# agent-charon/MinGraph-UNet

Measured on AMD Instinct MI355X. Metric: segmented Mpix/sec, full MinGraph-UNet forward (U-Net + patch-graph GAT), 512x512 batch, higher is better.
Workload: dtype f32

## Files before the change

### mingraph-unet_amd/csrc/common.h

```cpp
#pragma once
#include <hip/hip_runtime.h>
#include <stdint.h>

#include "device.h"

namespace mgu {

inline int grid_for(int64_t work, int threads, int cap) {
  int64_t b = (work + threads - 1) / threads;
  if (b < 1) b = 1;
  if (b > cap) b = cap;
  return (int)b;
}
inline bool aligned16(const void* p) { return ((uintptr_t)p & 15) == 0; }

struct Tuning {
  bool first_mfma = true;
  bool use_wino = true;
  int wino_prec = 1;
  bool convt_frag = true;
  bool wino_cp = true;
  int wino_ppb_cap = 32;
  bool wgrad_halo = true;
  bool wino_wgrad = true;
  bool convt_dgrad_x3 = true;
  bool wgrad_x3 = true;
  bool wgrad_thin = true;
  bool wino_dgrad = true;
  bool gat_fused = true;
  bool head_fused = true;
  bool wino_asm = true;
};
const Tuning& default_tuning();
hipError_t ensure_dyn_lds(const void* func, size_t bytes, bool (&done)[64]);

struct IgemmDesc {
  const Tuning* tn;
  const float* in;
  const float* w;
  const float* wu;
  const float* scale;
  const float* shift;
  float* out;
  int M;
  int H, W;
  int Cp;
  int ldin;
  int KS;
  int K;
  int Kp;
  int N;
  int ldout;
  int coff;
  int relu;
  int out_mode;
  int ct_cout;
  int Hout, Wout;
  float* pool;
  int ldpool;
  double* stat_slots;
  int split_n;
  float* out2;
  int ld2;
};

struct WinoHead {
  const float* w;
  const float* b;
  float* logits;
  float* psum;
  int ncls;
  int psum_bytes;
};
inline size_t wino_head_psum_bytes(int B, int H, int W) { return (size_t)B * (H / 16) * (W / 16) * 8 * 32 * sizeof(float); }

inline const Tuning& tun(const IgemmDesc& d) { return d.tn ? *d.tn : default_tuning(); }
enum class ConvKernel {
  None,
  WinoAsmWide, WinoAsmCp1r2, WinoAsmCp1r4,
  WinoAsmCp1r2Head,
  WinoCp2, WinoCp1, WinoCp2Stats, WinoCp1Stats,
  WinoCp1Head,
  WinoF32Wide, WinoF32Narrow,
  WinoX3Wide, WinoX3Narrow,
  HaloF32, HaloBf16Np8, HaloBf16Np4,
  TilesF32, TilesBf16,
  ConvtX3, ConvtBf16f, ConvtX3Dgrad,
};
ConvKernel pick_conv(const IgemmDesc& d, int dtype, const WinoHead* head = nullptr);
hipError_t launch_conv(const IgemmDesc& d, ConvKernel k, int dtype, hipStream_t s, const WinoHead* head = nullptr);
inline bool conv_fuses_head(ConvKernel k) { return k == ConvKernel::WinoAsmCp1r2Head || k == ConvKernel::WinoCp1Head; }
inline hipError_t launch_igemm_f32(const IgemmDesc& d, hipStream_t s) { return launch_conv(d, pick_conv(d, 0), 0, s); }
inline hipError_t launch_igemm_bf16(const IgemmDesc& d, hipStream_t s) { return launch_conv(d, pick_conv(d, 1), 1, s); }
const char* conv_kernel_name(ConvKernel k, const IgemmDesc& d);
const char* conv_dgrad_name(ConvKernel k, const IgemmDesc& d);
struct ConvCost {
  double mfma;
  int pipe;
};
ConvCost conv_cost(ConvKernel k, const IgemmDesc& d);
inline bool conv_is_wino(ConvKernel k) { return k >= ConvKernel::WinoAsmWide && k <= ConvKernel::WinoX3Narrow; }
inline bool conv_fuses_pool(ConvKernel k) {
  return conv_is_wino(k) || (k >= ConvKernel::HaloF32 && k <= ConvKernel::HaloBf16Np4);
}
inline bool conv_reads_panel(ConvKernel k) {
  return !conv_is_wino(k) && k != ConvKernel::ConvtX3 && k != ConvKernel::ConvtBf16f && k != ConvKernel::ConvtX3Dgrad;
}
bool wino_layer(const Tuning& t, int KS, int Cp);
bool wino_dgrad_layer(const Tuning& t, int KS, int Cop);
bool convt_x3_layer(const Tuning& t, int Cin, int Cout);
bool convt_x3_dgrad_layer(const Tuning& t, int Cin, int Cout);
bool convt_bf16f_layer(const Tuning& t, int Cin, int Cout);
bool wino_head_layer(const Tuning& t, int dtype, int Cin, int ncls, int patch, int B, int H, int W);
inline bool wino_wide(const IgemmDesc& d) { return d.N > 32; }
// ... 157 lines not shown
```

### mingraph-unet_amd/csrc/ctx.h

```cpp
#pragma once
#include <stdarg.h>
#include <stdio.h>
#include <stdlib.h>
#include <string.h>

#include <map>
#include <string>
#include <vector>

#include "../../include/mgunet.h"
#include "common.h"

struct Layer {
  std::string prefix;
  std::string conv;
  std::string bn;
  int Cin = 0, Cp = 0, Cout = 0, KS = 3;
  bool convt = false;
  int K = 0, Kp = 0, N = 0, Np = 0;
  float *wp = nullptr, *scale = nullptr, *shift = nullptr;
  bool first = false;
  bool ctb = false;
  bool ctx3 = false;
  bool wino = false;
// ... 11 lines not shown
  float *mean = nullptr, *invstd = nullptr, *tscale = nullptr, *tshift = nullptr;
  const float* t_in = nullptr;
  int t_ldin = 0;
  float* t_z = nullptr;
  float* t_y = nullptr;
  int t_ldy = 0;
  int t_B = 0, t_H = 0, t_W = 0;
  int level = 0;
};

struct Block {
  int up = -1;
  int conv1 = 0, conv2 = 0;
  int level = 0;
};

struct mgu_ctx {
  int device = 0;
  mgu::Tuning tn;
  std::string err;
  bool configured = false, loaded = false;
  std::vector<mgu::PackBatch> pack_host;
  mgu::PackBatch* pack_dev = nullptr;
  int pack_dev_cap = 0;
  bool want_train = false;
  bool fold_dirty = false;
  int* err_word = nullptr;
  void* redws = nullptr;
  size_t redws_bytes = 0;
  int last_stat_rows = 0;
  void* pm_out = nullptr;
  int pm_patch = 0;
  void* pmws = nullptr;
  size_t pmws_bytes = 0;
  void* wuws = nullptr;
  size_t wuws_bytes = 0;
  unsigned long long* gmaxbuf = nullptr;
  int gmax_cap = 0;
  unsigned gmax_gen = 0;
  struct mgu_gat_weights* gat_tmp = nullptr;
  void* lossws = nullptr;
  size_t lossws_bytes = 0;
  void* imgws = nullptr;
  size_t imgws_bytes = 0;
  void* ncws = nullptr;
  size_t ncws_bytes = 0;
  void* objws = nullptr;
  size_t objws_bytes = 0;
  int in_ch = 0, ncls = 0, feat = 0, depth = 0, dtype = 0, Cp0 = 0;
  std::vector<Layer> layers;
  std::vector<Block> enc, dec;
  Block bott;
  int head = 0;
  int64_t nparams = 0;
  float* arena = nullptr;
  size_t arena_floats = 0;
  void* ws = nullptr;
  size_t ws_bytes = 0;
  void* gbws = nullptr;
  size_t gbws_bytes = 0;
  void* gws = nullptr;
  size_t gws_bytes = 0;
  void* tws = nullptr;
  size_t tws_bytes = 0;
  bool have_train_fwd = false;
  int tB = 0, tH = 0, tW = 0;
  std::vector<float*> t_cat, t_feat, t_pooled;
  float* t_logits = nullptr;
  void* comm = nullptr;
  int comm_world = 1, comm_rank = 0;
  hipStream_t comm_stream = nullptr;
  hipEvent_t comm_ev[16] = {};
  int comm_ev_next = 0;
  bool prof = false;
  std::vector<hipEvent_t> ev;
  struct ProfRec {
    const char* name;
    double alg, mfma;
    int pipe;
  };
  std::vector<ProfRec> prec;
  int ev_used = 0;
  hipEvent_t ev_total[2] = {nullptr, nullptr};
};

namespace mgud {

inline int rup(int v, int m) { return (v + m - 1) / m * m; }
extern std::string g_create_err;

inline int fail(mgu_ctx* c, int code, const char* fmt, ...) {
  char buf[512];
  va_list ap;
  va_start(ap, fmt);
  vsnprintf(buf, sizeof buf, fmt, ap);
  va_end(ap);
  if (c) c->err = buf; else g_create_err = buf;
  return code;
}

#define HIPCHK(c, call)                                                                                       \
  do {                                                                                                        \
    hipError_t e_ = (call);                                                                                   \
    if (e_ != hipSuccess) return mgud::fail(c, MGU_ERR_HIP, "%s failed: %s", #call, hipGetErrorString(e_));   \
  } while (0)

inline int ensure(mgu_ctx* c, void** p, size_t* have, size_t need) {
  if (*have >= need) return MGU_OK;
  if (*p) {
    HIPCHK(c, hipDeviceSynchronize());
    HIPCHK(c, hipFree(*p));
    *p = nullptr;
    *have = 0;
  }
  hipError_t e = hipMalloc(p, need);
  if (e != hipSuccess) return fail(c, MGU_ERR_NOMEM, "hipMalloc(%zu) failed: %s", need, hipGetErrorString(e));
  *have = need;
  return MGU_OK;
}

inline int err_word_dev(mgu_ctx* c, int** dev) {
  if (!c->err_word) {
    HIPCHK(c, hipHostMalloc((void**)&c->err_word, sizeof(int), hipHostMallocMapped));
    *c->err_word = 0;
  }
  HIPCHK(c, hipHostGetDevicePointer((void**)dev, c->err_word, 0));
  return MGU_OK;
}
inline const char* err_word_message(int w) {
  return (w & 2) ? "the GAT backward found no edge whose score equals the forward's graph-wide maximum (mgu_gat_layer_backward): its "
                   "max term was not applied"
                 : "a label outside [0, num_classes) (and != ignore_index -100) reached a loss kernel of this context (mgu_cross_entropy / "
                   "mgu_dice_loss; F.one_hot / CrossEntropyLoss raise on it)";
}

struct Carve {
  size_t off = 0;
  size_t take(size_t bytes) {
    const size_t o = off;
    off += (bytes + 255) / 256 * 256;
    return o;
  }
};

struct ProfScope {
  mgu_ctx* c;
  hipStream_t s;
  int idx = -1;
  ProfScope(mgu_ctx* c_, hipStream_t s_, const char* name = "conv/GEMM", double alg = 0, double mfma = 0, int pipe = -1) : c(c_), s(s_) {
    if (!c || !c->prof) return;
    if ((size_t)c->ev_used >= c->prec.size()) c->prec.resize(c->ev_used + 1);
    c->prec[c->ev_used] = {name, alg, mfma, pipe};
    if ((size_t)(2 * c->ev_used + 2) > c->ev.size()) {
      hipEvent_t a, b;
      if (hipEventCreate(&a) != hipSuccess || hipEventCreate(&b) != hipSuccess) return;
      c->ev.push_back(a);
      c->ev.push_back(b);
    }
    idx = c->ev_used++;
    (void)hipEventRecord(c->ev[2 * idx], s);
  }
  ~ProfScope() {
    if (idx >= 0) (void)hipEventRecord(c->ev[2 * idx + 1], s);
  }
};

// ... 112 lines not shown
```

### mingraph-unet_amd/csrc/mgunet_api.hip

```cpp
#include "ctx.h"

#include <algorithm>

using namespace mgu;
using namespace mgud;

namespace mgud {
std::string g_create_err;
}

namespace {

struct WsPlan {
  size_t xin, tmp, bott, total;
  std::vector<size_t> pooled;
};

WsPlan plan_ws(const mgu_ctx* c, int B, int H, int W) {
  std::vector<int> hs, wsz;
  level_dims(H, W, c->depth, hs, wsz);
  auto out = [&](const Block& b, int l) { return (size_t)B * hs[l] * wsz[l] * c->layers[b.conv2].Cout; };
  WsPlan p;
  Carve k;
  const size_t es = c->dtype == MGU_DTYPE_BF16 ? 2 : 4;
  p.xin = k.take((size_t)B * H * W * c->Cp0 * es);
  size_t tmax = out(c->bott, c->bott.level);
  for (const Block& b : c->enc) tmax = std::max(tmax, out(b, b.level));
  p.tmp = k.take(tmax * es);
  for (const Block& b : c->enc) p.pooled.push_back(k.take(out(b, b.level + 1) * es));
  p.bott = k.take(out(c->bott, c->bott.level) * es);
  p.total = k.off;
  return p;
}

template <class F>
void weight_forms(const mgu_ctx* c, Layer& L, F form) {
  const int dtype = c->dtype;
  L.wino = dtype == MGU_DTYPE_F32 && !L.convt && wino_layer(c->tn, L.KS, L.Cp);
  L.ctx3 = dtype == MGU_DTYPE_F32 && L.convt && convt_x3_layer(c->tn, L.Cin, L.Cout);
  L.ctb = dtype == MGU_DTYPE_BF16 && L.convt && convt_bf16f_layer(c->tn, L.Cin, L.Cout);
  L.first = !L.convt && L.KS == 3 && first_conv_applicable(dtype, L.Cin, L.Cp, L.Cout, 8, 0);
  form(L.wp, (size_t)L.Np * L.Kp);
  form(L.scale, (size_t)L.Np);
  form(L.shift, (size_t)L.Np);
  if (L.wino) form(L.wu, wino_u_floats(L.Cout, L.Cp));
  if (L.wino && rup(L.Cout, 4) % 16 == 0) form(L.wug, wino_u_floats(L.Cin, rup(L.Cout, 4)));
  if (L.ctx3) form(L.wu, convt_x3_floats(L.Cin, L.Cout));
  if (L.ctb) form(L.wu, convt_bf16f_floats(L.Cin, L.Cout));
  if (L.ctx3) form(L.wxg, convt_x3_dgrad_floats(L.Cin, L.Cout));
  if (dtype == MGU_DTYPE_F32 && !L.convt && L.bn.empty())
    form(L.wxg, (size_t)rup(L.Cin, 128) * rup(L.KS * L.KS * rup(L.Cout, 4), 32));
  if (L.first) form(L.wf, 9 * 4 * (size_t)L.Cout);
  if (L.first) form(L.wfm, first_mfma_floats());
  if (!L.bn.empty()) {
    form(L.mean, (size_t)L.Np);
    form(L.invstd, (size_t)L.Np);
    form(L.tscale, (size_t)L.Np);
    form(L.tshift, (size_t)L.Np);
  }
}

}

extern "C" {

const char* mgu_version(void) { return "mgunet 0.2 (gfx950: fp32 Winograd / bf16 MFMA forward, fp32 training step, GAT, RCCL gradient exchange)"; }

int mgu_create(int device_id, mgu_ctx** out) {
  if (!out) return fail(nullptr, MGU_ERR_INVALID, "out == NULL");
  int n = 0;
  hipError_t e = hipGetDeviceCount(&n);
  if (e != hipSuccess || n <= 0)
    return fail(nullptr, MGU_ERR_HIP, "no HIP device available (%s): libmgunet has no CPU fallback",
                e != hipSuccess ? hipGetErrorString(e) : "device count 0");
  if (device_id < 0 || device_id >= n) return fail(nullptr, MGU_ERR_INVALID, "device %d out of range [0,%d)", device_id, n);
  e = hipSetDevice(device_id);
  if (e != hipSuccess) return fail(nullptr, MGU_ERR_HIP, "hipSetDevice: %s", hipGetErrorString(e));
  mgu_ctx* c = new mgu_ctx();
  c->device = device_id;
  auto flag = [](const char* name) { const char* v = getenv(name); return v && v[0] == '1'; };
  auto num = [](const char* name, int dflt) { const char* v = getenv(name); return v && v[0] ? atoi(v) : dflt; };
  Tuning& t = c->tn;
  t.first_mfma = !flag("MGU_NO_FIRST_MFMA");
  t.use_wino = !flag("MGU_NO_WINOGRAD");
  t.wino_prec = num("MGU_WINO_PREC", t.wino_prec) ? 1 : 0;
  t.wino_cp = !flag("MGU_NO_WINO_CP");
  t.convt_frag = !flag("MGU_NO_CONVT_FRAG");
  t.wino_ppb_cap = std::max(1, num("MGU_WINO_PPB_CAP", 32));
  t.wgrad_halo = !flag("MGU_NO_WGRAD_HALO");
  t.wino_wgrad = !flag("MGU_NO_WINO_WGRAD");
  t.wgrad_x3 = !flag("MGU_NO_WGRAD_X3");
  t.convt_dgrad_x3 = !flag("MGU_NO_CONVT_DGRAD_X3");
  t.wgrad_thin = !flag("MGU_NO_THIN_WGRAD");
  t.wino_dgrad = !flag("MGU_NO_WINO_DGRAD");
  t.gat_fused = !flag("MGU_NO_GAT_FUSED");
  t.wino_asm = num("MGU_WINO_ASM", 1) > 0;
  t.head_fused = num("MGU_HEAD_FUSED", 1) > 0;
  *out = c;
  return MGU_OK;
}

void mgu_destroy(mgu_ctx* c) {
  if (!c) return;
  (void)hipSetDevice(c->device);
  (void)hipDeviceSynchronize();
  (void)mgu_comm_destroy(c);
  if (c->arena) (void)hipFree(c->arena);
  if (c->ws) (void)hipFree(c->ws);
  if (c->gws) (void)hipFree(c->gws);
  if (c->pmws) (void)hipFree(c->pmws);
  if (c->gbws) (void)hipFree(c->gbws);
  if (c->pack_dev) (void)hipFree(c->pack_dev);
  if (c->tws) (void)hipFree(c->tws);
  if (c->redws) (void)hipFree(c->redws);
  if (c->wuws) (void)hipFree(c->wuws);
  if (c->ncws) (void)hipFree(c->ncws);
  if (c->objws) (void)hipFree(c->objws);
  if (c->lossws) (void)hipFree(c->lossws);
  if (c->imgws) (void)hipFree(c->imgws);
  gat_destroy(c);
  if (c->err_word) (void)hipHostFree(c->err_word);
  for (auto e : c->ev) (void)hipEventDestroy(e);
  for (auto e : c->ev_total)
    if (e) (void)hipEventDestroy(e);
  delete c;
}

const char* mgu_last_error(mgu_ctx* c) { return c ? c->err.c_str() : g_create_err.c_str(); }

int mgu_unet_configure(mgu_ctx* c, int in_ch, int ncls, int feat, int depth, int dtype) {
  if (!c) return MGU_ERR_INVALID;
  if (in_ch < 1 || ncls < 1 || feat < 4 || (feat & 3) || depth < 1 || depth > 8)
    return fail(c, MGU_ERR_INVALID, "unsupported UNet(%d,%d,%d,%d): init_features must be a positive multiple of 4, depth 1..8",
                in_ch, ncls, feat, depth);
  if (dtype != MGU_DTYPE_F32 && dtype != MGU_DTYPE_BF16) return fail(c, MGU_ERR_INVALID, "unknown dtype %d", dtype);
  if (dtype == MGU_DTYPE_BF16 && ((feat & 7) || ncls > 4))
    return fail(c, MGU_ERR_INVALID, "bf16 storage needs init_features %% 8 == 0 (16-byte lanes of 8 bf16) and <= 4 classes");
  HIPCHK(c, hipSetDevice(c->device));
  c->in_ch = in_ch, c->ncls = ncls, c->feat = feat, c->depth = depth, c->dtype = dtype;
  c->Cp0 = rup(in_ch, dtype == MGU_DTYPE_BF16 ? 8 : 4);
  c->layers.clear();
  c->enc.clear();
  c->dec.clear();
  auto add = [&](const std::string& prefix, const char* conv, const char* bn, int cin, int cp, int cout, int KS, bool convt, int level) {
    Layer L;
    L.prefix = prefix, L.conv = conv, L.bn = bn;
    L.Cin = cin, L.Cp = cp, L.Cout = cout, L.KS = KS, L.convt = convt, L.level = level;
    c->layers.push_back(L);
    return (int)c->layers.size() - 1;
  };
  auto add_block = [&](const std::string& prefix, int cin, int cp, int cout, int level, int up) {
    Block b;
    b.up = up, b.level = level;
    b.conv1 = add(prefix, "conv1", "bn1", cin, cp, cout, 3, false, level);
    b.conv2 = add(prefix, "conv2", "bn2", cout, cout, cout, 3, false, level);
    return b;
  };
  int cin = in_ch, cp = c->Cp0, f = feat;
  for (int i = 0; i < depth; ++i) {
    c->enc.push_back(add_block("encoder.encoder_blocks." + std::to_string(i) + ".", cin, cp, f, i, -1));
    cin = cp = f;
    f *= 2;
  }
  c->bott = add_block("encoder.bottleneck.", cin, cp, f, depth, -1);
  int prev = f;
  for (int b = 0; b < depth; ++b) {
    const int i = depth - 1 - b, ci = feat << i;
    const std::string prefix = "decoder.decoder_blocks." + std::to_string(b) + ".";
    const int up = add(prefix, "upsample", "", prev, prev, prev / 2, 1, true, i + 1);
    c->dec.push_back(add_block(prefix + "conv_block.", ci + prev / 2, ci + prev / 2, ci, i, up));
    prev = ci;
  }
  c->head = add("decoder.", "final_conv", "", prev, prev, ncls, 1, false, 0);
  for (auto& L : c->layers) {
    L.K = L.KS * L.KS * L.Cp;
    L.Kp = rup(L.K, dtype == MGU_DTYPE_BF16 ? 64 : 32);
    L.N = L.convt ? 4 * L.Cout : L.Cout;
    L.Np = rup(L.N, 128);
  }
  {
    int64_t off = 0;
    auto conv = [&](Layer& L) {
      L.off_w = off, off += (int64_t)L.Cout * L.Cin * L.KS * L.KS * (L.convt ? 4 : 1);
      L.off_b = off, off += L.Cout;
    };
    auto bn = [&](Layer& L) {
      L.off_gamma = off, off += L.Cout;
      L.off_beta = off, off += L.Cout;
    };
    auto block = [&](const Block& b) {
      if (b.up >= 0) conv(c->layers[b.up]);
      conv(c->layers[b.conv1]), conv(c->layers[b.conv2]);
      bn(c->layers[b.conv1]), bn(c->layers[b.conv2]);
    };
    for (const Block& b : c->enc) block(b);
    block(c->bott);
    for (const Block& b : c->dec) block(b);
    conv(c->layers[c->head]);
    c->nparams = off;
  }
  size_t total = 0;
  for (auto& L : c->layers) weight_forms(c, L, [&](float*&, size_t n) { total += n; });
  if (c->arena) HIPCHK(c, hipFree(c->arena));
  c->arena = nullptr;
  HIPCHK(c, hipMalloc((void**)&c->arena, total * sizeof(float)));
  HIPCHK(c, hipMemset(c->arena, 0, total * sizeof(float)));
  c->arena_floats = total;
// ... 119 lines not shown
        items.push_back(pack_wino(w, L.wug, L.Cin, L.Cout, rup(L.Cout, 4), 1, c->tn.wino_prec));
        L.wug_valid = true;
      }
      const bool head_kernel = L.bn.empty() && c->ncls <= 4;
      if (!L.wu && !L.first && !head_kernel) {
        items.push_back(pack_conv_panel(w, L.wp, c->dtype, L.Cout, L.Cin, L.Cp, L.KS, L.Kp));
        L.wp_dirty = false;
      }
      if (L.wf) items.push_back(pack_first_w(w, L.wf, L.Cout, L.Cin));
      if (L.wfm && L.Cout == 32 && L.Cin <= 3) items.push_back(pack_first_mfma(w, L.wfm, L.Cout, L.Cin));
      if (!L.bn.empty()) c->fold_dirty = true;
      else items.push_back(pack_bias_tile(b, L.shift, L.Cout, 1));
      if (L.bn.empty() && L.wxg && c->want_train) {
        const int Cop = rup(L.Cout, 4);
        items.push_back(pack_dgrad_panel(w, L.wxg, L.Cout, L.Cin, Cop, L.KS, rup(L.KS * L.KS * Cop, 32)));
        L.wxg_valid = true;
      }
    }
  }
  std::vector<PackBatch> batches;
  for (size_t i0 = 0; i0 < items.size(); i0 += PACK_MAX) {
    PackBatch b;
    memset(&b, 0, sizeof b);
    b.n = (int)std::min<size_t>(PACK_MAX, items.size() - i0);
    for (int i = 0; i < b.n; ++i) b.it[i] = items[i0 + i];
    if (!pack_batch_prepare(b)) return fail(c, MGU_ERR_STATE, "internal: a weight form is not packable");
    batches.push_back(b);
  }
  const bool same = batches.size() == c->pack_host.size() &&
                    (batches.empty() || memcmp(batches.data(), c->pack_host.data(), batches.size() * sizeof(PackBatch)) == 0);
  if (!same) {
    if ((int)batches.size() > c->pack_dev_cap) {
      if (c->pack_dev) HIPCHK(c, hipFree(c->pack_dev));
      c->pack_dev = nullptr;
      HIPCHK(c, hipMalloc((void**)&c->pack_dev, batches.size() * sizeof(PackBatch)));
      c->pack_dev_cap = (int)batches.size();
    }
    HIPCHK(c, hipStreamSynchronize(s));
    HIPCHK(c, hipMemcpy(c->pack_dev, batches.data(), batches.size() * sizeof(PackBatch), hipMemcpyHostToDevice));
    c->pack_host = batches;
  }
  for (size_t k = 0; k < batches.size(); ++k) HIPCHK(c, launch_pack_batch(c->pack_dev + k, batches[k].total_blocks, s));
  return MGU_OK;
}

int mgud::run_layer(mgu_ctx* c, const Layer& L, const void* in_v, int ldin, int B, int H, int W, void* out_v, int ldout,
                    int coff, int relu, const float* scale, const float* shift, int Hout, int Wout, hipStream_t s,
                    void* pool, int ldpool, bool* pool_fused, double* stat_slots, bool* stat_fused, const WinoHead* head,
                    bool* head_fused) {
  IgemmDesc d = layer_desc(c, L, in_v, ldin, B, H, W, out_v, ldout, coff);
  if (head_fused) *head_fused = false;
  d.scale = scale, d.shift = shift, d.relu = relu, d.Hout = Hout, d.Wout = Wout;
  if (pool_fused) *pool_fused = false;
  if (stat_fused) *stat_fused = false;
  if (L.wfm && c->tn.first_mfma && ldin == L.Cp && first_mfma_applicable(c->dtype, L.Cin, L.Cp, L.Cout, ldout, coff, H, W)) {
    const double alg = 2.0 * d.M * 9.0 * L.Cin * L.Cout;
    ProfScope ps(c, s, "conv3x3_first_mfma_kernel", alg, 2.0 * d.M * 32.0 * 32.0 * (c->dtype == MGU_DTYPE_F32 ? 6.0 : 3.0), 1);
    HIPCHK(c, launch_first_mfma(c->dtype, in_v, L.wfm, scale, shift, out_v, B, H, W, ldout, coff, relu, s));
    return MGU_OK;
  }
  if (L.wf && ldin == L.Cp && first_conv_applicable(c->dtype, L.Cin, L.Cp, L.Cout, ldout, coff) &&
      (int64_t)B * H * W * std::max(ldout, 8) < (1ll << 31)) {
    ProfScope ps(c, s, "conv3x3_first_kernel", 2.0 * d.M * 9.0 * L.Cin * L.Cout, 0, -1);
    HIPCHK(c, launch_first_conv(c->dtype, in_v, L.wf, scale, shift, out_v, B, H, W, L.Cin, L.Cout, ldout, coff, relu, s));
    return MGU_OK;
  }
  ConvKernel k = pick_conv(d, c->dtype, head);
  if (stat_slots && conv_is_wino(k) && wino_grid_blocks(d) <= STAT_ROWS) {
    d.stat_slots = stat_slots;
    c->last_stat_rows = wino_grid_blocks(d);
    if (stat_fused) *stat_fused = true;
  }
  if (pool && conv_fuses_pool(k)) {
    d.pool = (float*)pool, d.ldpool = ldpool;
    if (pool_fused) *pool_fused = true;
  }
  if (d.stat_slots || d.pool) k = pick_conv(d, c->dtype, head);
  if (!conv_fuses_head(k)) head = nullptr;
  else if (head_fused) *head_fused = true;
  if (L.wp_dirty && conv_reads_panel(k)) {
    HIPCHK(c, launch_pack_one(L.convt ? pack_convt_panel(L.w_src, L.wp, c->dtype, L.Cin, L.Cout, L.Kp)
                                      : pack_conv_panel(L.w_src, L.wp, c->dtype, L.Cout, L.Cin, L.Cp, L.KS, L.Kp), s));
    L.wp_dirty = false;
  }
  double alg = L.convt ? 2.0 * d.M * (double)L.Cin * L.Cout * 4.0 : 2.0 * d.M * (double)L.KS * L.KS * L.Cin * L.Cout;
  if (head) alg += 2.0 * d.M * (double)L.Cout * head->ncls;
  const ConvCost cost = conv_cost(k, d);
  ProfScope ps(c, s, conv_kernel_name(k, d), alg, cost.mfma, cost.pipe);
  HIPCHK(c, launch_conv(d, k, c->dtype, s, head));
  return MGU_OK;
}

static int run_conv(mgu_ctx* c, const Layer& L, const void* in, int ldin, int B, int H, int W, void* out, int ldout,
                    int coff, int relu, int Hout, int Wout, hipStream_t s, void* pool = nullptr, int ldpool = 0,
                    bool* pool_fused = nullptr, const WinoHead* head = nullptr, bool* head_fused = nullptr) {
  return run_layer(c, L, in, ldin, B, H, W, out, ldout, coff, relu, L.bn.empty() ? nullptr : L.scale, L.shift, Hout, Wout, s,
                   pool, ldpool, pool_fused, nullptr, nullptr, head, head_fused);
}

extern "C" {

int mgu_unet_forward(mgu_ctx* c, const void* x_dev, int B, int H, int W, int64_t xs_n, int64_t xs_c, int64_t xs_h,
                     int64_t xs_w, void* logits_dev, void* const* cat_dev, void* const* feat_dev, int training,
                     void* hip_stream) {
  if (!c) return MGU_ERR_INVALID;
  if (!c->configured || !c->loaded) return fail(c, MGU_ERR_STATE, "configure + load_weights must precede forward");
  if (!x_dev || !logits_dev || !cat_dev || !feat_dev) return fail(c, MGU_ERR_INVALID, "NULL buffer");
  const int depth = c->depth;
  if (B < 1 || H < (1 << depth) || W < (1 << depth))
    return fail(c, MGU_ERR_INVALID, "input %dx%dx%d too small for depth %d", B, H, W, depth);
  if ((int64_t)B * H * W >= (1ll << 31)) return fail(c, MGU_ERR_INVALID, "B*H*W must be < 2^31");
  for (int i = 0; i < depth; ++i)
    if (!cat_dev[i] || !feat_dev[i]) return fail(c, MGU_ERR_INVALID, "NULL cat/feat buffer %d", i);
  HIPCHK(c, hipSetDevice(c->device));
  hipStream_t s = (hipStream_t)hip_stream;
  if (training && c->dtype != MGU_DTYPE_F32)
    return fail(c, MGU_ERR_STATE, "training runs in fp32 only (bf16 storage is an inference mode)");
  if (training) {
    int rc = unet_forward_train(c, (const float*)x_dev, xs_n, xs_c, xs_h, xs_w, B, H, W, (float*)logits_dev, cat_dev, feat_dev, s);
    if (rc == MGU_OK && c->pm_out) {
      ProfScope ps(c, s, "patch_mean_kernel", 0, 0, -1);
      HIPCHK(c, launch_patch_mean(feat_dev[0], 0, (float*)c->pm_out, B, H, W, c->feat, c->pm_patch, s));
      c->pm_out = nullptr;
    }
    return rc;
  }
  const WsPlan plan = plan_ws(c, B, H, W);
  int rc = ensure(c, &c->ws, &c->ws_bytes, plan.total);
  if (rc) return rc;
  const Layer& F = c->layers[c->head];
  WinoHead head_args{};
  bool head_done = false;
  const bool head_wanted = c->pm_out && F.w_src && F.b_src && wino_head_layer(c->tn, c->dtype, F.Cin, c->ncls, c->pm_patch, B, H, W);
  if (head_wanted) {
    if ((rc = ensure(c, &c->pmws, &c->pmws_bytes, wino_head_psum_bytes(B, H, W)))) return rc;
    head_args = WinoHead{F.w_src, F.b_src, (float*)logits_dev, (float*)c->pmws, c->ncls, (int)wino_head_psum_bytes(B, H, W)};
  }
  if (c->fold_dirty) {
    for (auto& L : c->layers)
      if (!L.bn.empty()) HIPCHK(c, launch_bn_fold(L.b_src, L.gamma, L.beta, L.run_mean, L.run_var, 1e-5f, L.scale, L.shift, L.Cout, s));
    c->fold_dirty = false;
  }
  char* ws = (char*)c->ws;
  const size_t es = c->dtype == MGU_DTYPE_BF16 ? 2 : 4;
  void* xin = ws + plan.xin;
  void* tmp = ws + plan.tmp;
  void* bott = ws + plan.bott;
  std::vector<int> hs, wsz;
  level_dims(H, W, depth, hs, wsz);

  if (c->prof) {
    for (auto& e : c->ev_total)
      if (!e) HIPCHK(c, hipEventCreate(&e));
    HIPCHK(c, hipEventRecord(c->ev_total[0], s));
  }

  for (const Block& b : c->enc) {
    const int i = b.level;
    if (2 * hs[i + 1] != hs[i] || 2 * wsz[i + 1] != wsz[i])
      HIPCHK(c, hipMemsetAsync(cat_dev[i], 0, (size_t)B * hs[i] * wsz[i] * 2 * c->layers[b.conv2].Cout * es, s));
  }

  const Layer& L0 = c->layers[c->enc[0].conv1];
  const bool first_direct = L0.wfm && c->tn.first_mfma && first_mfma_applicable(c->dtype, L0.Cin, L0.Cp, L0.Cout, c->feat, 0, H, W) &&
                            (int64_t)B * H * W < (1ll << 31);
  if (!first_direct) HIPCHK(c, launch_pack_input((const float*)x_dev, xin, c->dtype, B, c->in_ch, c->Cp0, H, W, xs_n, xs_c, xs_h, xs_w, s));

  const void* cur = xin;
  int cur_ld = c->Cp0;
  for (const Block& b : c->enc) {
    const int i = b.level, C = c->layers[b.conv1].Cout;
    if (&b == &c->enc.front() && first_direct) {
      if (c->fold_dirty) return fail(c, MGU_ERR_STATE, "internal: eval scale/shift not folded");
      const double alg = 2.0 * B * H * W * 9.0 * L0.Cin * L0.Cout;
      ProfScope ps(c, s, "conv3x3_first_mfma_kernel", alg, 2.0 * B * H * W * 32.0 * 32.0 * (c->dtype == MGU_DTYPE_F32 ? 6.0 : 3.0), 1);
      HIPCHK(c, launch_first_mfma_direct(c->dtype, (const float*)x_dev, xs_n, xs_c, xs_h, xs_w, c->in_ch, L0.wfm, L0.bn.empty() ? nullptr : L0.scale,
                                         L0.shift, tmp, B, H, W, C, 0, 1, s));
    } else if ((rc = run_conv(c, c->layers[b.conv1], cur, cur_ld, B, hs[i], wsz[i], tmp, C, 0, 1, 0, 0, s))) return rc;
    void* pooled = ws + plan.pooled[i];
    bool fused = false;
    if ((rc = run_conv(c, c->layers[b.conv2], tmp, C, B, hs[i], wsz[i], cat_dev[i], 2 * C, 0, 1, 0, 0, s, pooled, C, &fused))) return rc;
    if (!fused) HIPCHK(c, launch_maxpool2(cat_dev[i], 2 * C, pooled, c->dtype, B, hs[i], wsz[i], C, s));
    cur = pooled;
    cur_ld = C;
  }
  {
    const Block& b = c->bott;
    const int i = b.level, C = c->layers[b.conv1].Cout;
    if ((rc = run_conv(c, c->layers[b.conv1], cur, cur_ld, B, hs[i], wsz[i], tmp, C, 0, 1, 0, 0, s))) return rc;
    if ((rc = run_conv(c, c->layers[b.conv2], tmp, C, B, hs[i], wsz[i], bott, C, 0, 1, 0, 0, s))) return rc;
    cur = bott;
    cur_ld = C;
  }
  for (const Block& b : c->dec) {
    const int i = b.level, C = c->layers[b.conv1].Cout;
    const bool last = head_wanted && i == 0;
    if ((rc = run_conv(c, c->layers[b.up], cur, cur_ld, B, hs[i + 1], wsz[i + 1], cat_dev[i], 2 * C, C, 0, hs[i], wsz[i], s)))
      return rc;
    if ((rc = run_conv(c, c->layers[b.conv1], cat_dev[i], 2 * C, B, hs[i], wsz[i], tmp, C, 0, 1, 0, 0, s))) return rc;
    if ((rc = run_conv(c, c->layers[b.conv2], tmp, C, B, hs[i], wsz[i], feat_dev[i], C, 0, 1, 0, 0, s, nullptr, 0, nullptr,
                       last ? &head_args : nullptr, last ? &head_done : nullptr)))
      return rc;
    cur = feat_dev[i];
    cur_ld = C;
  }
  {
    const int pm_dtype = c->dtype;
    if (head_done) {
      ProfScope ps(c, s, "patch_sum_combine_kernel", 0, 0, -1);
      HIPCHK(c, launch_patch_sum_combine((const float*)c->pmws, (float*)c->pm_out, B * (H / 16) * (W / 16), s));
      c->pm_out = nullptr;
    } else if (c->pm_out && F.w_src && F.b_src && patch_mean_head_fusable(pm_dtype, F.Cin, c->ncls) && F.Cin <= 256) {
      ProfScope ps(c, s, "patch_mean_kernel (1x1 head + patch means)", 2.0 * B * H * W * F.Cin * c->ncls, 0, -1);
      HIPCHK(c, launch_patch_mean(cur, pm_dtype, (float*)c->pm_out, B, H, W, F.Cin, c->pm_patch, s, F.w_src, F.b_src,
                                  (float*)logits_dev, c->ncls));
      c->pm_out = nullptr;
    } else if (c->ncls <= 4 && F.w_src && F.b_src) {
      ProfScope ps(c, s, "conv1x1_head_kernel", 2.0 * B * H * W * F.Cin * c->ncls, 0, -1);
      HIPCHK(c, launch_conv1x1_head(cur, c->dtype, cur_ld, F.Cin, F.w_src, F.b_src, (float*)logits_dev, c->ncls, c->ncls,
                                    (int64_t)B * H * W, s));
    } else if ((rc = run_conv(c, F, cur, cur_ld, B, H, W, logits_dev, c->ncls, 0, 0, 0, 0, s))) {
      return rc;
    }
  }
  if (c->pm_out) {
    ProfScope ps(c, s, "patch_mean_kernel", 0, 0, -1);
    HIPCHK(c, launch_patch_mean(cur, c->dtype, (float*)c->pm_out, B, H, W, F.Cin, c->pm_patch, s));
    c->pm_out = nullptr;
  }
  if (c->prof) HIPCHK(c, hipEventRecord(c->ev_total[1], s));
  return MGU_OK;
}

int mgu_unet_request_patch_mean(mgu_ctx* c, int patch, void* out_dev) {
  if (!c) return MGU_ERR_INVALID;
  if (!c->configured) return fail(c, MGU_ERR_STATE, "not configured");
  if (!out_dev) {
    c->pm_out = nullptr;
    return MGU_OK;
  }
  if (patch < 1) return fail(c, MGU_ERR_INVALID, "bad patch_mean request");
  const int C = c->layers[c->head].Cin, vec = c->dtype == MGU_DTYPE_BF16 ? 8 : 4;
  if ((C % vec) || C > 256) return fail(c, MGU_ERR_INVALID, "patch means need init_features %% %d == 0 and <= 256 (got %d)", vec, C);
  c->pm_patch = patch;
  c->pm_out = out_dev;
  return MGU_OK;
}

struct mgu_conv_weights {
  Layer L;
};

static Layer block_layer(int Cin, int Cout, int ksize, bool convt) {
  Layer L;
  L.Cin = L.Cp = Cin, L.Cout = Cout, L.KS = ksize, L.convt = convt;
  L.K = ksize * ksize * Cin, L.Kp = rup(L.K, 32), L.N = convt ? 4 * Cout : Cout, L.Np = rup(L.N, 128);
  return L;
}

static int conv2d_launch(mgu_ctx* c, const Layer& L, const void* in_dev, int B, int H, int W, const void* bias_dev, const void* scale_dev,
                         const void* shift_dev, int relu, void* out_dev, int ld_out, int c_off, hipStream_t s) {
  IgemmDesc d = layer_desc(c, L, in_dev, L.Cin, B, H, W, out_dev, ld_out, c_off);
  d.relu = relu;
  if (scale_dev && shift_dev) {
    d.scale = (const float*)scale_dev;
    d.shift = (const float*)shift_dev;
  } else if (bias_dev) {
    HIPCHK(c, launch_pack_one(pack_bias_tile((const float*)bias_dev, L.shift, L.Cout, 1), s));
    d.shift = L.shift;
  }
  const ConvKernel k = pick_conv(d, 0);
  ProfScope ps(c, s, conv_kernel_name(k, d));
  HIPCHK(c, launch_conv(d, k, 0, s));
  return MGU_OK;
}

int mgu_conv2d_prepare(mgu_ctx* c, const void* w_dev, int Cout, int Cin, int ksize, mgu_conv_weights** out, void* hip_stream) {
  if (!c) return MGU_ERR_INVALID;
  if (!w_dev || !out || Cout < 1 || (ksize != 1 && ksize != 3)) return fail(c, MGU_ERR_INVALID, "bad conv2d_prepare args (ksize must be 1 or 3)");
  if (Cin < 4 || (Cin & 3)) return fail(c, MGU_ERR_INVALID, "conv2d needs Cin %% 4 == 0 (got %d)", Cin);
  HIPCHK(c, hipSetDevice(c->device));
  hipStream_t s = (hipStream_t)hip_stream;
  mgu_conv_weights* p = new mgu_conv_weights();
  Layer& L = p->L;
  L = block_layer(Cin, Cout, ksize, false);
  const bool wino = wino_layer(c->tn, ksize, Cin);
  const size_t panel = (size_t)L.Np * L.Kp, total = panel + L.Np + (wino ? wino_u_floats(Cout, Cin) : 0);
  hipError_t e = hipMalloc((void**)&L.wp, total * sizeof(float));
// ... 195 lines not shown
```

Measured before the change: 804.6.

## Split U-Net forward batch into two image groups on concurrent streams

Splits the batch into two halves and runs the encoder/decoder walk for each half on its own stream (the main stream plus a new non-blocking stream), with per-group tmp slices and offset activation pointers, joined by events. The aim is to overlap kernels from the two groups so small, low-occupancy layers at deep levels fill the GPU better and launch gaps are hidden. In exchange each kernel gets half the work, which can lower per-kernel efficiency on the large layers. It also adds event synchronisation, including an extra wait when weight panels are repacked during the first group.

Measured after the change: 821.0, median of 6. +2.0%, better.

```diff
diff --git a/mingraph-unet_amd/csrc/common.h b/mingraph-unet_amd/csrc/common.h
--- a/mingraph-unet_amd/csrc/common.h
+++ b/mingraph-unet_amd/csrc/common.h
@@ -30,6 +30,7 @@
   bool gat_fused = true;
   bool head_fused = true;
   bool wino_asm = true;
+  int fwd_groups = 2;
 };
 const Tuning& default_tuning();
 hipError_t ensure_dyn_lds(const void* func, size_t bytes, bool (&done)[64]);
diff --git a/mingraph-unet_amd/csrc/ctx.h b/mingraph-unet_amd/csrc/ctx.h
--- a/mingraph-unet_amd/csrc/ctx.h
+++ b/mingraph-unet_amd/csrc/ctx.h
@@ -117,6 +117,9 @@
   std::vector<ProfRec> prec;
   int ev_used = 0;
   hipEvent_t ev_total[2] = {nullptr, nullptr};
+  hipStream_t fwd_stream = nullptr;
+  hipEvent_t fwd_ev[2] = {nullptr, nullptr};
+  int panel_packs = 0;
 };
 
 namespace mgud {
diff --git a/mingraph-unet_amd/csrc/mgunet_api.hip b/mingraph-unet_amd/csrc/mgunet_api.hip
--- a/mingraph-unet_amd/csrc/mgunet_api.hip
+++ b/mingraph-unet_amd/csrc/mgunet_api.hip
@@ -12,9 +12,12 @@
 namespace {
 
 struct WsPlan {
-  size_t xin, tmp, bott, total;
+  size_t xin, tmp, tmp_slice, bott, total;
   std::vector<size_t> pooled;
 };
+
+int fwd_groups(const mgu_ctx* c, int B) { return c->tn.fwd_groups >= 2 && B >= 2 ? 2 : 1; }
+int group_images(const mgu_ctx* c, int B) { return (B + fwd_groups(c, B) - 1) / fwd_groups(c, B); }
 
 WsPlan plan_ws(const mgu_ctx* c, int B, int H, int W) {
   std::vector<int> hs, wsz;
@@ -26,7 +29,9 @@
   p.xin = k.take((size_t)B * H * W * c->Cp0 * es);
   size_t tmax = out(c->bott, c->bott.level);
   for (const Block& b : c->enc) tmax = std::max(tmax, out(b, b.level));
-  p.tmp = k.take(tmax * es);
+  const int G = fwd_groups(c, B);
+  p.tmp_slice = (tmax / B * group_images(c, B) * es + 255) / 256 * 256;
+  p.tmp = k.take(G == 1 ? tmax * es : G * p.tmp_slice);
   for (const Block& b : c->enc) p.pooled.push_back(k.take(out(b, b.level + 1) * es));
   p.bott = k.take(out(c->bott, c->bott.level) * es);
   p.total = k.off;
@@ -96,6 +101,7 @@
   t.gat_fused = !flag("MGU_NO_GAT_FUSED");
   t.wino_asm = num("MGU_WINO_ASM", 1) > 0;
   t.head_fused = num("MGU_HEAD_FUSED", 1) > 0;
+  t.fwd_groups = num("MGU_FWD_GROUPS", t.fwd_groups) >= 2 ? 2 : 1;
   *out = c;
   return MGU_OK;
 }
@@ -123,6 +129,9 @@
   for (auto e : c->ev) (void)hipEventDestroy(e);
   for (auto e : c->ev_total)
     if (e) (void)hipEventDestroy(e);
+  for (auto e : c->fwd_ev)
+    if (e) (void)hipEventDestroy(e);
+  if (c->fwd_stream) (void)hipStreamDestroy(c->fwd_stream);
   delete c;
 }
 
@@ -408,6 +417,7 @@
     HIPCHK(c, launch_pack_one(L.convt ? pack_convt_panel(L.w_src, L.wp, c->dtype, L.Cin, L.Cout, L.Kp)
                                       : pack_conv_panel(L.w_src, L.wp, c->dtype, L.Cout, L.Cin, L.Cp, L.KS, L.Kp), s));
     L.wp_dirty = false;
+    ++c->panel_packs;
   }
   double alg = L.convt ? 2.0 * d.M * (double)L.Cin * L.Cout * 4.0 : 2.0 * d.M * (double)L.KS * L.KS * L.Cin * L.Cout;
   if (head) alg += 2.0 * d.M * (double)L.Cout * head->ncls;
@@ -470,7 +480,6 @@
   char* ws = (char*)c->ws;
   const size_t es = c->dtype == MGU_DTYPE_BF16 ? 2 : 4;
   void* xin = ws + plan.xin;
-  void* tmp = ws + plan.tmp;
   void* bott = ws + plan.bott;
   std::vector<int> hs, wsz;
   level_dims(H, W, depth, hs, wsz);
@@ -492,44 +501,79 @@
                             (int64_t)B * H * W < (1ll << 31);
   if (!first_direct) HIPCHK(c, launch_pack_input((const float*)x_dev, xin, c->dtype, B, c->in_ch, c->Cp0, H, W, xs_n, xs_c, xs_h, xs_w, s));
 
-  const void* cur = xin;
-  int cur_ld = c->Cp0;
-  for (const Block& b : c->enc) {
-    const int i = b.level, C = c->layers[b.conv1].Cout;
-    if (&b == &c->enc.front() && first_direct) {
-      if (c->fold_dirty) return fail(c, MGU_ERR_STATE, "internal: eval scale/shift not folded");
-      const double alg = 2.0 * B * H * W * 9.0 * L0.Cin * L0.Cout;
-      ProfScope ps(c, s, "conv3x3_first_mfma_kernel", alg, 2.0 * B * H * W * 32.0 * 32.0 * (c->dtype == MGU_DTYPE_F32 ? 6.0 : 3.0), 1);
-      HIPCHK(c, launch_first_mfma_direct(c->dtype, (const float*)x_dev, xs_n, xs_c, xs_h, xs_w, c->in_ch, L0.wfm, L0.bn.empty() ? nullptr : L0.scale,
-                                         L0.shift, tmp, B, H, W, C, 0, 1, s));
-    } else if ((rc = run_conv(c, c->layers[b.conv1], cur, cur_ld, B, hs[i], wsz[i], tmp, C, 0, 1, 0, 0, s))) return rc;
-    void* pooled = ws + plan.pooled[i];
-    bool fused = false;
-    if ((rc = run_conv(c, c->layers[b.conv2], tmp, C, B, hs[i], wsz[i], cat_dev[i], 2 * C, 0, 1, 0, 0, s, pooled, C, &fused))) return rc;
-    if (!fused) HIPCHK(c, launch_maxpool2(cat_dev[i], 2 * C, pooled, c->dtype, B, hs[i], wsz[i], C, s));
-    cur = pooled;
-    cur_ld = C;
-  }
-  {
-    const Block& b = c->bott;
-    const int i = b.level, C = c->layers[b.conv1].Cout;
-    if ((rc = run_conv(c, c->layers[b.conv1], cur, cur_ld, B, hs[i], wsz[i], tmp, C, 0, 1, 0, 0, s))) return rc;
-    if ((rc = run_conv(c, c->layers[b.conv2], tmp, C, B, hs[i], wsz[i], bott, C, 0, 1, 0, 0, s))) return rc;
-    cur = bott;
-    cur_ld = C;
-  }
-  for (const Block& b : c->dec) {
-    const int i = b.level, C = c->layers[b.conv1].Cout;
-    const bool last = head_wanted && i == 0;
-    if ((rc = run_conv(c, c->layers[b.up], cur, cur_ld, B, hs[i + 1], wsz[i + 1], cat_dev[i], 2 * C, C, 0, hs[i], wsz[i], s)))
-      return rc;
-    if ((rc = run_conv(c, c->layers[b.conv1], cat_dev[i], 2 * C, B, hs[i], wsz[i], tmp, C, 0, 1, 0, 0, s))) return rc;
-    if ((rc = run_conv(c, c->layers[b.conv2], tmp, C, B, hs[i], wsz[i], feat_dev[i], C, 0, 1, 0, 0, s, nullptr, 0, nullptr,
-                       last ? &head_args : nullptr, last ? &head_done : nullptr)))
-      return rc;
-    cur = feat_dev[i];
-    cur_ld = C;
-  }
+  auto walk = [&](hipStream_t gs, int img0, int nb, void* tmp, bool* head_done) -> int {
+    auto at = [&](const void* base, int level, int ch) { return (char*)base + (size_t)img0 * hs[level] * wsz[level] * ch * es; };
+    WinoHead head = head_args;
+    if (head_wanted) {
+      head.logits += (size_t)img0 * H * W * c->ncls;
+      head.psum = (float*)((char*)head.psum + wino_head_psum_bytes(img0, H, W));
+      head.psum_bytes = (int)wino_head_psum_bytes(nb, H, W);
+    }
+    const void* cur = at(xin, 0, c->Cp0);
+    int cur_ld = c->Cp0;
+    for (const Block& b : c->enc) {
+      const int i = b.level, C = c->layers[b.conv1].Cout;
+      if (&b == &c->enc.front() && first_direct) {
+        if (c->fold_dirty) return fail(c, MGU_ERR_STATE, "internal: eval scale/shift not folded");
+        const double alg = 2.0 * nb * H * W * 9.0 * L0.Cin * L0.Cout;
+        ProfScope ps(c, gs, "conv3x3_first_mfma_kernel", alg, 2.0 * nb * H * W * 32.0 * 32.0 * (c->dtype == MGU_DTYPE_F32 ? 6.0 : 3.0), 1);
+        HIPCHK(c, launch_first_mfma_direct(c->dtype, (const float*)x_dev + (int64_t)img0 * xs_n, xs_n, xs_c, xs_h, xs_w, c->in_ch, L0.wfm,
+                                           L0.bn.empty() ? nullptr : L0.scale, L0.shift, tmp, nb, H, W, C, 0, 1, gs));
+      } else if ((rc = run_conv(c, c->layers[b.conv1], cur, cur_ld, nb, hs[i], wsz[i], tmp, C, 0, 1, 0, 0, gs))) return rc;
+      void* pooled = at(ws + plan.pooled[i], i + 1, C);
+      bool fused = false;
+      if ((rc = run_conv(c, c->layers[b.conv2], tmp, C, nb, hs[i], wsz[i], at(cat_dev[i], i, 2 * C), 2 * C, 0, 1, 0, 0, gs, pooled, C, &fused)))
+        return rc;
+      if (!fused) HIPCHK(c, launch_maxpool2(at(cat_dev[i], i, 2 * C), 2 * C, pooled, c->dtype, nb, hs[i], wsz[i], C, gs));
+      cur = pooled;
+      cur_ld = C;
+    }
+    {
+      const Block& b = c->bott;
+      const int i = b.level, C = c->layers[b.conv1].Cout;
+      if ((rc = run_conv(c, c->layers[b.conv1], cur, cur_ld, nb, hs[i], wsz[i], tmp, C, 0, 1, 0, 0, gs))) return rc;
+      if ((rc = run_conv(c, c->layers[b.conv2], tmp, C, nb, hs[i], wsz[i], at(bott, i, C), C, 0, 1, 0, 0, gs))) return rc;
+      cur = at(bott, i, C);
+      cur_ld = C;
+    }
+    for (const Block& b : c->dec) {
+      const int i = b.level, C = c->layers[b.conv1].Cout;
+      const bool last = head_wanted && i == 0;
+      if ((rc = run_conv(c, c->layers[b.up], cur, cur_ld, nb, hs[i + 1], wsz[i + 1], at(cat_dev[i], i, 2 * C), 2 * C, C, 0, hs[i], wsz[i], gs)))
+        return rc;
+      if ((rc = run_conv(c, c->layers[b.conv1], at(cat_dev[i], i, 2 * C), 2 * C, nb, hs[i], wsz[i], tmp, C, 0, 1, 0, 0, gs))) return rc;
+      if ((rc = run_conv(c, c->layers[b.conv2], tmp, C, nb, hs[i], wsz[i], at(feat_dev[i], i, C), C, 0, 1, 0, 0, gs, nullptr, 0, nullptr,
+                         last ? &head : nullptr, last ? head_done : nullptr)))
+        return rc;
+      cur = at(feat_dev[i], i, C);
+      cur_ld = C;
+    }
+    return MGU_OK;
+  };
+  const int G = c->prof ? 1 : fwd_groups(c, B);
+  if (G == 1) {
+    if ((rc = walk(s, 0, B, ws + plan.tmp, &head_done))) return rc;
+  } else {
+    if (!c->fwd_stream) HIPCHK(c, hipStreamCreateWithFlags(&c->fwd_stream, hipStreamNonBlocking));
+    for (auto& e : c->fwd_ev)
+      if (!e) HIPCHK(c, hipEventCreateWithFlags(&e, hipEventDisableTiming));
+    const int n0 = group_images(c, B), packs = c->panel_packs;
+    bool done1 = false;
+    HIPCHK(c, hipEventRecord(c->fwd_ev[0], s));
+    HIPCHK(c, hipStreamWaitEvent(c->fwd_stream, c->fwd_ev[0], 0));
+    rc = walk(s, 0, n0, ws + plan.tmp, &head_done);
+    if (rc == MGU_OK && c->panel_packs != packs) {
+      HIPCHK(c, hipEventRecord(c->fwd_ev[0], s));
+      HIPCHK(c, hipStreamWaitEvent(c->fwd_stream, c->fwd_ev[0], 0));
+    }
+    const int rc1 = rc == MGU_OK ? walk(c->fwd_stream, n0, B - n0, ws + plan.tmp + plan.tmp_slice, &done1) : MGU_OK;
+    HIPCHK(c, hipEventRecord(c->fwd_ev[1], c->fwd_stream));
+    HIPCHK(c, hipStreamWaitEvent(s, c->fwd_ev[1], 0));
+    if (rc || rc1) return rc ? rc : rc1;
+    if (done1 != head_done) return fail(c, MGU_ERR_STATE, "internal: the image groups disagree on the head-fused kernel");
+  }
+  const void* cur = feat_dev[0];
+  const int cur_ld = c->layers[c->dec.back().conv1].Cout;
   {
     const int pm_dtype = c->dtype;
     if (head_done) {
```
